# kit4b/kit4b

Measured on AMD Instinct MI355X. Metric: Mreads/sec aligned (100 bp SE vs 3 Gbp .sfx), higher is better.
Workload: dtype u64

## Files before the change

kit4b_amd/__init__.py:

```python
import ctypes as C
import os
import subprocess

import numpy as np

PKG_DIR = os.path.dirname(os.path.abspath(__file__))
LIB_PATH = os.path.join(PKG_DIR, os.environ.get("K4SFX_LIB_NAME", "libk4sfx.so"))

STRAND_BOTH, STRAND_WATSON, STRAND_CRICK = 0, 1, 2
HR_NONE, HR_HITS, HR_MMDELTA, HR_HITINSTS, HR_RMMDELTA, HR_SEQERRS = 0, 1, 2, 3, 4, 5
NAR_ACCEPTED, NAR_NS, NAR_NOHIT, NAR_MMDELTA, NAR_MULTIALIGN = 1, 2, 3, 4, 5

HIT_DTYPE = np.dtype(
    [("chrom_id", "<u4"), ("match_loci", "<u4"), ("match_len", "<u2"), ("strand", "u1"), ("mismatches", "u1"),
     ("reserved", "<u4")]
)
RESULT_DTYPE = np.dtype(
    [("hit_rslt", "<i4"), ("inst", "<i4"), ("low_mm", "<i4"), ("nxt_mm", "<i4"), ("nar", "<i4"), ("num_hits", "<i4")]
)
EXT_CHIMERIC, EXT_INDEL, EXT_INSERT, EXT_SPLICE, EXT_NONORPHAN = 1 << 24, 1 << 25, 1 << 26, 1 << 27, 1 << 28
SEG2_DTYPE = np.dtype(
    [("chrom_id", "<u4"), ("match_loci", "<u4"), ("match_len", "<u2"), ("read_ofs", "<u2"), ("mismatches", "u1"),
     ("reserved", "u1"), ("score", "<u2")]
)
# ... 231 lines not shown
                                        C.POINTER(u64), C.POINTER(SamStats), vp, vp]
    L.k4_format_bam_dev.argtypes = [vp, i32, i64, vp, vp, C.c_int32, vp, vp, vp, vp, vp, C.POINTER(SamNames), C.c_int32, C.POINTER(vp),
                                    C.POINTER(u64), C.POINTER(SamStats), vp, vp]
    L.k4_pipeline_format_bam.argtypes = [vp, C.c_int32, C.POINTER(SamStats), vp, C.POINTER(u64)]
    L.k4_pipeline_open.argtypes = [vp, C.POINTER(PipelineParams), C.POINTER(vp)]
    L.k4_pipeline_acquire.argtypes = [vp, i32, C.POINTER(vp), C.POINTER(u64)]
    L.k4_pipeline_submit.argtypes = [vp, i32, u64, i32]
    L.k4_pipeline_submit_host.argtypes = [vp, i32, vp, u64, i32]
    L.k4_pipeline_wait_aligned.argtypes = [vp, C.POINTER(PipelineView)]
    L.k4_pipeline_format.argtypes = [vp, C.POINTER(SamStats), vp, C.POINTER(u64)]
    L.k4_pipeline_next_sam.argtypes = [vp, C.POINTER(vp), C.POINTER(u64)]
    L.k4_pipeline_read_sam.argtypes = [vp, vp, u64, C.POINTER(u64)]
    L.k4_pipeline_close.argtypes = [vp]
    L.k4_pipeline_close.restype = None
    L.k4_free_device.argtypes = [vp]
    L.k4_free_device.restype = None
    L.k4_alloc_device.argtypes = [vp, u64, C.POINTER(vp)]
    L.k4_copy_to_device.argtypes = [vp, vp, vp, u64]
    L.k4_copy_to_host.argtypes = [vp, vp, vp, u64]
    L.k4_upload_pageable.argtypes = [i32, vp, vp, u64]
    L.k4_host_register.argtypes = [vp, u64]
    L.k4_host_unregister.argtypes = [vp]
    dbl, pvp, pu64 = C.c_double, C.POINTER(vp), C.POINTER(u64)
    fmt_head = [vp, i32, i64, vp, vp, C.c_int32, vp, vp, vp, vp, vp, C.POINTER(SamNames)]
    L.k4_format_sam_all_dev.argtypes = fmt_head + [pvp, pu64, C.POINTER(SamStats), vp, vp]
    L.k4_format_bam_all_dev.argtypes = fmt_head + [C.c_int32, pvp, pu64, C.POINTER(SamStats), vp, vp]
    L.k4_pipeline_format_all.argtypes = [vp, C.POINTER(SamStats), vp, pu64]
    L.k4_pipeline_format_bam_all.argtypes = [vp, C.c_int32, C.POINTER(SamStats), vp, pu64]
    L.k4_pipeline_set_trims.argtypes = [vp, C.c_int32, C.c_int32]
    L.k4_pipeline_set_sampling.argtypes = [vp, C.c_int32]
    L.k4_unaligned_fasta_dev.argtypes = [vp, i32, i64, vp, vp, vp, vp, vp, C.POINTER(SamNames), C.c_int32, pvp, pu64, pu64, vp]
    L.k4_prepare_reads_trim_dev.argtypes = [vp, i32, i64, C.c_int32, C.c_int32, C.c_int32, C.c_int32, C.c_int32, i64, vp, vp, vp, vp, u64,
                                            vp, vp, pu64, pu64, C.POINTER(u32), vp]
    snp_head = [vp, i32, i64, vp, vp, C.c_int32, vp, vp, vp, vp, C.c_int32, dbl, dbl]
    L.k4_snp_csv_dev.argtypes = snp_head + [pvp, pu64, pu64, vp]
    L.k4_snp_vcf_dev.argtypes = snp_head + [pvp, pu64, pu64, vp]
    L.k4_snp_files_dev.argtypes = [vp, i32] + snp_head[1:] + [pvp, pu64, pu64, pvp, pu64, vp]
    L.k4_snp_run_dev.argtypes = [vp, i32] + snp_head[1:] + [vp, vp]
    L.k4_snp_run2_dev.argtypes = [vp, i32] + snp_head[1:] + [C.POINTER(SnpOpts), C.POINTER(SnpFiles2), vp]
    L.k4_marker_classify_host.argtypes = [vp, u64, u32, vp, C.c_int32, dbl, vp, vp]
    L.k4_free_host.argtypes = [vp]
    L.k4_free_host.restype = None
    L.k4_pba_run_dev.argtypes = [vp, i32, i64, vp, vp, C.c_int32, vp, vp, vp, vp, C.c_char_p, C.c_char_p, C.POINTER(PbaFiles), vp]
    L.k4_pba_classify_host.argtypes = [vp, u64, u32, vp, vp, vp]
    L.k4_sfx_map.argtypes = [C.c_char_p, vp]
    L.k4_sfx_unmap.argtypes = [vp]
    L.k4_sfx_unmap.restype = None
    L.k4_set_raw_header.argtypes = [vp, vp]
    L.k4_set_description.argtypes = [vp, C.c_char_p, C.c_char_p]
    L.k4_get_sfx_header.argtypes = [vp, vp]
    L.k4_abi_version.argtypes = []
    L.k4_global_error.argtypes = []
    L.k4_get_kernel_times_split.argtypes = [vp, C.POINTER(dbl), C.POINTER(dbl), C.POINTER(C.c_int32)]
    _lib = L
    return L


def _flatten(reads):
    if isinstance(reads, tuple):
        cat, offs, lens = reads
        return (np.ascontiguousarray(cat, dtype=np.uint8), np.ascontiguousarray(offs, dtype=np.uint64),
                np.ascontiguousarray(lens, dtype=np.uint32))
    lens = np.array([len(r) for r in reads], dtype=np.uint32)
    offs = np.zeros(len(reads), dtype=np.uint64)
    if len(reads):
        offs[1:] = np.cumsum(lens[:-1], dtype=np.uint64)
        cat = np.ascontiguousarray(np.concatenate(reads).astype(np.uint8))
    else:
        cat = np.zeros(0, dtype=np.uint8)
    return cat, offs, lens


def gen_hash16(name):
    if not name:
        return 0
    h = 19937
    for ch in name.lower():
        h = ((h ^ ch) * 3119) & 0xFFFFFFFF
        if h & 0x80000000:
            h -= 1 << 32
        h ^= h >> 13
        h &= 0xFFFF
    return h or 19937


def make_entries(names, lens):
    arr = (Entry * len(names))()
    ofs = 0
    for i, (nm, ln) in enumerate(zip(names, lens)):
        arr[i].entry_id = i + 1
        arr[i].fblock_id = 1
        arr[i].name = nm.encode() if isinstance(nm, str) else nm
        arr[i].name_hash = gen_hash16(arr[i].name)
        arr[i].seq_len = int(ln)
        arr[i].start_ofs = ofs
        arr[i].end_ofs = ofs + int(ln) - 1
        ofs += int(ln) + 1
    return arr


class SfxIndex:

    def __init__(self, handle):
        self.h = C.c_void_p(handle)
        self._keep = []

# ... 40 lines not shown
    def info(self):
        o = Info()
        self._ck(lib().k4_info(self.h, C.byref(o)))
        return {f[0]: (getattr(o, f[0]).decode() if f[0] == "dataset" else getattr(o, f[0])) for f in Info._fields_}

    def entry(self, entry_id):
        e = Entry()
        self._ck(lib().k4_get_entry(self.h, entry_id, C.byref(e)))
        return dict(entry_id=e.entry_id, name=e.name.decode(), seq_len=e.seq_len, start_ofs=e.start_ofs,
                    end_ofs=e.end_ofs)

    def get_ident(self, name):
        return lib().k4_get_ident(self.h, name.encode())

    def set_max_iter(self, it):
        return lib().k4_set_max_iter(self.h, it)

    def set_fastq_quality(self, method):
        self._ck(lib().k4_set_fastq_quality(self.h, method))

    def get_seq(self, entry_id, loci, length):
        out = np.zeros(length, dtype=np.uint8)
        n = lib().k4_get_seq(self.h, entry_id, loci, out.ctypes.data, length)
        return out[:n]

    def write_sfx(self, path):
        self._ck(lib().k4_write_sfx(self.h, path.encode()))

    def min_core_len(self, pmode=0):
        s = C.c_int(0)
        m = self._ck(lib().k4_min_core_len(self.h, pmode, C.byref(s)))
        return m, s.value

    def counters(self):
        c = Counters()
        self._ck(lib().k4_get_counters(self.h, C.byref(c)))
        return {f[0]: getattr(c, f[0]) for f in Counters._fields_}

    def reset_counters(self):
        self._ck(lib().k4_reset_counters(self.h))

    def enable_kernel_timing(self, on=True):
        self._ck(lib().k4_enable_kernel_timing(self.h, 1 if on else 0))

    def kernel_times(self):
        ms, n = C.c_double(0), C.c_int32(0)
        self._ck(lib().k4_get_kernel_times(self.h, C.byref(ms), C.byref(n)))
        return ms.value, n.value

    def kernel_times_split(self):
        ms, g, n = C.c_double(0), C.c_double(0), C.c_int32(0)
        self._ck(lib().k4_get_kernel_times_split(self.h, C.byref(ms), C.byref(g), C.byref(n)))
        return ms.value, g.value, n.value

    def reserve(self, max_reads, max_read_len, max_hits):
        self._ck(lib().k4_reserve(self.h, max_reads, max_read_len, max_hits))

    def align_reads_batch(self, reads, tot_mm, core_len, core_delta, max_slides, min_core_len=0, mm_delta=1,
                          strand=STRAND_BOTH, max_hits=1):
        cat, offs, lens = _flatten(reads)
        n = len(lens)
        p = AlignParams(tot_mm, core_len, core_delta, max_slides, min_core_len, mm_delta, strand, max_hits)
        rslt = np.zeros(n, np.int32); inst = np.zeros(n, np.int32); low = np.zeros(n, np.int32)
        nxt = np.zeros(n, np.int32)
        hits = np.zeros((n, max_hits), dtype=HIT_DTYPE)
        self._ck(lib().k4_align_reads_batch(self.h, C.byref(p), n, cat.ctypes.data, offs.ctypes.data,
                                            lens.ctypes.data, rslt.ctypes.data, inst.ctypes.data, low.ctypes.data,
                                            nxt.ctypes.data, hits.ctypes.data))
        return dict(rslt=rslt, inst=inst, low=low, nxt=nxt, hits=hits)

    def align_reads_ext_batch(self, reads, tot_mm, core_len, core_delta, max_slides, min_core_len=0, mm_delta=1,
                              strand=STRAND_BOTH, max_hits=1, min_chimeric_len=0, micro_indel_len=0, max_splice_junct_len=0):
        cat, offs, lens = _flatten(reads)
        n = len(lens)
        p = AlignParams(tot_mm, core_len, core_delta, max_slides, min_core_len, mm_delta, strand, max_hits,
                        min_chimeric_len, micro_indel_len, max_splice_junct_len)
        rslt = np.zeros(n, np.int32); inst = np.zeros(n, np.int32); low = np.zeros(n, np.int32)
        nxt = np.zeros(n, np.int32)
        hits = np.zeros((n, max_hits), dtype=HIT_DTYPE)
        seg2 = np.zeros(n, dtype=SEG2_DTYPE)
        self._ck(lib().k4_align_reads_ext_batch(self.h, C.byref(p), n, cat.ctypes.data, offs.ctypes.data, lens.ctypes.data,
                                                rslt.ctypes.data, inst.ctypes.data, low.ctypes.data, nxt.ctypes.data,
                                                hits.ctypes.data, seg2.ctypes.data))
        return dict(rslt=rslt, inst=inst, low=low, nxt=nxt, hits=hits, seg2=seg2)

    def kalign_ext_batch(self, reads, max_subs=5, min_edit_dist=1, max_ns=1, pmode=0, strand=STRAND_BOTH, max_ml=1,
                         pe_mode=0, min_core_len=0, max_num_slides=0, min_chimeric_len=0, micro_indel_len=0,
                         max_splice_junct_len=0):
        cat, offs, lens = _flatten(reads)
        n = len(lens)
        p = KalignParams(max_subs, min_edit_dist, max_ns, pmode, strand, max_ml, pe_mode, min_core_len, max_num_slides,
                         min_chimeric_len, micro_indel_len, max_splice_junct_len)
        out = np.zeros(n, dtype=RESULT_DTYPE)
        hits = np.zeros((n, max(1, max_ml)), dtype=HIT_DTYPE)
        seg2 = np.zeros(n, dtype=SEG2_DTYPE)
        self._ck(lib().k4_kalign_ext_batch(self.h, C.byref(p), n, cat.ctypes.data, offs.ctypes.data, lens.ctypes.data,
                                           out.ctypes.data, hits.ctypes.data, seg2.ctypes.data))
        return dict(out=out, hits=hits, seg2=seg2)

    def best_matches_batch(self, reads, tot_mm, core_len, core_delta, max_core_slides, strand=STRAND_BOTH, max_hits=5):
        cat, offs, lens = _flatten(reads)
        n = len(lens)
        p = AlignParams(tot_mm, core_len, core_delta, max_core_slides, 0, 1, strand, max_hits)
        rslt = np.zeros(n, dtype=np.int32)
        inst = np.zeros(n, dtype=np.int32)
        hits = np.zeros((n, max_hits), dtype=HIT_DTYPE)
# ... 473 lines not shown
```

kit4b_amd/csrc/k4_align.hip:

```cpp
#include <stdlib.h>
#include <type_traits>
#include "k4_align_common.h"

#define K4_BS(nch) ((nch) >= 16 ? 128 : 256)
template <int NCH>
struct K4Lane {
  const uint64_t* rd;
  uint32_t* ded;
  const uint32_t* sup;
  const uint64_t* ent;
  uint64_t* memo;
  static constexpr int NW = NCH + 1;
  K4_DEV uint64_t word(int s, int c) const { return rd[(s * NW + c) * K4_BS(NCH)]; }
  K4_DEV uint64_t chunk_at(int s, int o) const {
    int w = o >> 5, sh = 2 * (o & 31);
    uint64_t hi = word(s, w);
    if (!sh) return hi;
    return (hi << sh) | (word(s, w + 1) >> (64 - sh));
  }
};

struct K4Probe {
  int cmp;
  int mm;
// ... 273 lines not shown
    if (32 * c < len) {
      uint32_t dq[9] = {0, 0, 0, 0, 0, 0, 0, 0, 0};
      if (c * 32 + 32 <= span) {
        uint32_t d8[8];
        k4d_load_words<8>(src32 + c * 8, d8);
#pragma unroll
        for (int q = 0; q < 8; q++) dq[q] = d8[q];
      } else {
#pragma unroll
        for (int q = 0; q < 8; q++)
          if (c * 32 + q * 4 < span) dq[q] = src32[c * 8 + q];
      }
      if (c * 32 + 32 < span) dq[8] = src32[c * 8 + 8];
#pragma unroll
      for (int q = 0; q < 8; q++) {
        const int base = c * 32 + q * 4;
        uint32_t d = __builtin_amdgcn_alignbyte(dq[q + 1], dq[q], sh);
        d &= 0x07070707u;
        if (base + 4 > len) d &= len > base ? (0xFFFFFFFFu >> (8 * (4 - (len - base)))) : 0u;
        const uint32_t hi4 = d & 0x04040404u;
        if (hi4) {
          const uint32_t inval = hi4 & ((d << 1) | (d << 2)) & 0x04040404u;
          if (inval) fl |= K4_RF_INVALID;
          n_ns += __popc(hi4 & ~inval);
          d &= ~(hi4 | (hi4 >> 1) | (hi4 >> 2));
        }
        acc = (acc << 8) | ((d & 3) << 6) | (((d >> 8) & 3) << 4) | (((d >> 16) & 3) << 2) | ((d >> 24) & 3);
      }
    }
    col[c * K4_BS(NCH)] = acc;
  }
  col[NCH * K4_BS(NCH)] = 0;
  if (n_ns) fl |= K4_RF_HAS_N;
#pragma unroll
  for (int c = 0; c < NCH; c++) {
    uint64_t r = 0;
    if (32 * c < len) {
      const int o = len - 32 * (c + 1);
      uint64_t f;
      if (o >= 0) {
        const int w = o >> 5, sh = 2 * (o & 31);
        const uint64_t hi = col[w * K4_BS(NCH)];
        f = sh ? (hi << sh) | (col[(w + 1) * K4_BS(NCH)] >> (64 - sh)) : hi;
      } else
        f = col[0] >> (2 * (-o));
      r = k4d_rev2(~f) & k4d_range_mask(0, len - 32 * c);
    }
    col[(NW + c) * K4_BS(NCH)] = r;
  }
  col[(NW + NCH) * K4_BS(NCH)] = 0;
  return fl;
}

template <int EL, int NCH, bool FIRST, typename KT, bool DEFER = false>
__global__ void __launch_bounds__(K4_BS(NCH), (NCH >= 16 ? K4_STEP_WAVES_LONG : NCH >= 8 ? K4_STEP_WAVES_MID : NCH == 5 ? K4_STEP_WAVES_5 : K4_STEP_WAVES)) k4k_align_step(K4AlignArgs a, int step, const uint32_t* __restrict__ in_ids,
                                                      const uint64_t* __restrict__ in_rows,
                                                      const uint32_t* __restrict__ in_count, uint32_t* __restrict__ out_ids,
                                                      uint64_t* __restrict__ out_rows, uint32_t* __restrict__ out_count) {
  extern __shared__ uint64_t lds[];
  constexpr int NW = NCH + 1;
  const int tid = threadIdx.x;
  const int lane = tid & 63;
  K4Lane<NCH> ln;
  ln.rd = lds + tid;
  ln.ded = reinterpret_cast<uint32_t*>(lds + 2 * NW * K4_BS(NCH)) + tid;
  ln.memo = lds + 2 * NW * K4_BS(NCH) + (K4_DEDUP_CAP * K4_BS(NCH)) / 2 + tid;
  uint64_t* ent_l = lds + 2 * NW * K4_BS(NCH) + (K4_DEDUP_CAP * K4_BS(NCH)) / 2 + 2 * K4_BS(NCH);
  uint32_t* sup_l = reinterpret_cast<uint32_t*>(ent_l + 2 * K4_LDS_ENTRIES);
  ln.ent = ent_l;
  ln.sup = sup_l;
  for (int q = tid; q < K4_SUP_WORDS; q += K4_BS(NCH)) sup_l[q] = a.ix.excsup[q];
  if (a.ix.n_entries <= K4_LDS_ENTRIES)
    for (int q = tid; q < (int)a.ix.n_entries; q += K4_BS(NCH)) {
      ent_l[q] = a.ix.ent_start[q];
      ent_l[K4_LDS_ENTRIES + q] = a.ix.ent_end[q];
    }
  __syncthreads();
  uint64_t* col = lds + tid;
  uint32_t n_lookup = 0, n_probe = 0, n_cand = 0, n_slow = 0, n_bases = 0, n_done = 0;
  const int64_t count = (FIRST && !(DEFER && in_ids != nullptr)) ? a.n_reads : (int64_t)*in_count;
  const int64_t stride = (int64_t)gridDim.x * K4_BS(NCH);
  uint32_t ch_cur = 0, ch_left = 0;
  const bool from_list = !FIRST || (DEFER && in_ids != nullptr);
  const bool may_defer = DEFER && FIRST && in_ids == nullptr && a.defer_ids != nullptr;
  uint32_t dch_cur = 0, dch_left = 0;
  for (int64_t jb = (int64_t)blockIdx.x * K4_BS(NCH) + (tid & ~63); jb < count; jb += stride) {
    const int64_t j = jb + lane;
    bool active = j < count;
    int64_t i = 0;
    if (active) {
      i = from_list ? (int64_t)in_ids[j] : j;
      if (from_list && (uint32_t)i == K4_NO_READ) active = false;
    }
    bool slow = false, survive = false, deferred = false;
    int ext_from = -1;
    if (active) {
      const int len = (int)a.lens[i];
      const K4ReadParams rp = k4d_read_params(a, len);
      bool skip = false;
      if (FIRST) {
        if (!from_list) {
          n_done++;
          n_bases += (uint32_t)len;
        }
        uint32_t fl = 0, n_ns = 0;
        if (len < 1 || len > 32 * NCH || len > K4_MAX_FAST_READ_LEN) {
          fl = K4_RF_TOOLONG;
          if (a.mode == 1) {
            const uint8_t* src = a.reads + a.offs[i];
            for (int q = 0; q < len; q++) {
              uint32_t b = src[q] & 7;
              if (b == 4) n_ns++; else if (b > 4) fl |= K4_RF_INVALID;
            }
          }
        } else
          fl = k4d_pack_read<NCH>(a.reads + a.offs[i], len, col, n_ns);
        if (a.mode == 1) {
          int max_ns = 0;
          if (a.kp.max_ns) max_ns = max((len * a.kp.max_ns) / 100, a.kp.max_ns);
          if ((fl & K4_RF_INVALID) || (int)n_ns > max_ns) {
            k4_read_result r = {K4_HR_SEQERRS, 0, 0, 0, K4_NAR_NS, 0};
            a.rr[i] = r;
            if (!a.sparse_hits)
              for (int q = 0; q < a.max_hits; q++) *reinterpret_cast<uint4*>(&a.hits[i * a.max_hits + q]) = make_uint4(0, 0, 0, 0);
            skip = true;
          }
        }
        slow = fl != 0 && !skip;
        if (((a.mode == 1 && a.kp.pe_mode == 4) || a.best) && !skip) slow = true;
      } else {
        const uint64_t* row = in_rows + (int64_t)j * K4_ROW_WORDS(NCH);
        {
          const k4_u64x2_a8 mv = *reinterpret_cast<const k4_u64x2_a8*>(row + 2 * NCH);
          ln.memo[0] = mv.x; ln.memo[K4_BS(NCH)] = mv.y;
        }
        uint64_t rw[2 * NCH];
#pragma unroll
        for (int c = 0; c < NCH; c++) {
          const k4_u64x2_a8 v = *reinterpret_cast<const k4_u64x2_a8*>(row + 2 * c);
          rw[2 * c] = v.x; rw[2 * c + 1] = v.y;
        }
#pragma unroll
        for (int c = 0; c < NCH; c++) {
          col[c * K4_BS(NCH)] = rw[c];
          col[(NW + c) * K4_BS(NCH)] = rw[NCH + c];
        }
        col[NCH * K4_BS(NCH)] = 0;
        col[(NW + NCH) * K4_BS(NCH)] = 0;
      }
      if (!skip && (rp.core_len < 1 || rp.max_hits < 1 || rp.max_hits > a.max_hits)) slow = true;
      if (!skip && !slow) {
        int n_esc = 0;
        if (rp.tot_mm > 0)
          for (; n_esc <= rp.tot_mm; n_esc++)
            if (len / (n_esc + rp.mm_delta) <= rp.core_len) break;
        const bool has_final = rp.tot_mm > 0 ? n_esc <= rp.tot_mm : true;
        const int n_phases = n_esc + (has_final ? 1 : 0);
        int allow, cl, delta;
        if (step < n_esc) { allow = step; cl = len / (step + rp.mm_delta); delta = cl; }
        else { allow = rp.tot_mm; cl = rp.core_len; delta = rp.core_delta; }
        k4_hit* hits = a.hits + i * a.max_hits;
        int inst = 0, low = 0, nxt = 0;
        const uint32_t c0 = n_lookup, c1 = n_probe, c2 = n_cand;
        if (FIRST) { ln.memo[0] = K4_MEMO_NONE; ln.memo[K4_BS(NCH)] = K4_MEMO_NONE; }
        int rslt = k4d_lcm_fast<EL, NCH, KT, FIRST>(a, ln, len, allow, cl, delta, rp, &inst, &low, &nxt, hits, n_lookup, n_probe, n_cand, DEFER && may_defer);
        if (rslt == K4_NEED_SLOW) {
          slow = true;
          n_lookup = c0; n_probe = c1; n_cand = c2;
        }
        else if (DEFER && rslt == K4_DEFER) {
          deferred = true;
          n_lookup = c0; n_probe = c1; n_cand = c2;
        }
        else if (rslt == 0 && step + 1 >= n_phases && a.ext_on) { slow = true; ext_from = n_phases; }
        else if (rslt != 0 || step + 1 >= n_phases) k4d_finalize(a, i, len, rp, rslt, inst, low, nxt);
        else survive = true;
      }
      if (slow) {
        k4d_push_slow(a, i, ext_from >= 0 ? ext_from : step);
        n_slow++;
      }
    }
    if (FIRST && DEFER) {
      const unsigned long long dm = __ballot(deferred);
      const uint32_t dcnt = (uint32_t)__popcll(dm);
      if (dcnt) {
        if (dcnt > dch_left) {
          for (uint32_t q = lane; q < dch_left; q += 64) a.defer_ids[dch_cur + q] = K4_NO_READ;
          uint32_t base = 0;
          if (lane == 0) base = atomicAdd(&a.ctl[K4_CTL_DEFER], (uint32_t)K4_CHUNK);
          dch_cur = __shfl(base, 0, 64);
          dch_left = K4_CHUNK;
        }
        if (deferred) a.defer_ids[dch_cur + (uint32_t)__popcll(dm & ((1ull << lane) - 1ull))] = (uint32_t)i;
        dch_cur += dcnt;
        dch_left -= dcnt;
      }
    }
    const unsigned long long m = __ballot(survive);
    const uint32_t cnt = (uint32_t)__popcll(m);
    if (cnt) {
      if (cnt > ch_left) {
        for (uint32_t q = lane; q < ch_left; q += 64) out_ids[ch_cur + q] = K4_NO_READ;
        uint32_t base = 0;
        if (lane == 0) base = atomicAdd(out_count, (uint32_t)K4_CHUNK);
        ch_cur = __shfl(base, 0, 64);
        ch_left = K4_CHUNK;
      }
      if (survive) {
        const uint32_t slot = ch_cur + (uint32_t)__popcll(m & ((1ull << lane) - 1ull));
        out_ids[slot] = (uint32_t)i;
        uint64_t* row = out_rows + (int64_t)slot * K4_ROW_WORDS(NCH);
#pragma unroll
// ... 56 lines not shown
  int fast_len = std::min<int>(max_read_len, K4_MAX_FAST_READ_LEN);
  if (max_reads > w.cap_reads || fast_len > w.cap_len) {
    int64_t cap = std::max<int64_t>(max_reads, w.cap_reads);
    cap = (cap + 255) / 256 * 256;
    int len = std::max(fast_len, w.cap_len);
    int nch = nch_for(len);
    touched = true;
    w.cap_reads = 0;
    w.cap_len = 0;
    const size_t slots = k4_survivor_slots((size_t)cap);
    for (int b = 0; b < 2; b++) {
      K4_HIP(ix, w.ids[b].reserve(slots * 4));
      K4_HIP(ix, w.rows[b].reserve(slots * K4_ROW_WORDS(nch) * 8));
    }
    K4_HIP(ix, w.slow_list.reserve((size_t)cap * 4));
    K4_HIP(ix, w.slow_step.reserve((size_t)cap));
    K4_HIP(ix, w.huge_list.reserve((size_t)cap * 4));
    K4_HIP(ix, w.huge_step.reserve((size_t)cap));
    w.cap_reads = cap;
    w.cap_len = len;
  }
  if (!w.ctl.p) {
    touched = true;
    K4_HIP(ix, w.ctl.reserve(K4_CTL_WORDS * 4));
    K4_HIP(ix, hipMemset(w.ctl.p, 0, K4_CTL_WORDS * 4));
  }
  uint64_t nodes = ix->d.max_iter ? std::min<uint64_t>((uint64_t)ix->d.max_iter * 48, K4_MAX_IDENT_NODES) : K4_MAX_IDENT_NODES;
  uint32_t hcap = next_pow2(std::max<uint64_t>(2 * nodes + 2, 1024));
  if (!w.slow_hash.p || hcap > w.slow_hash_cap) {
    touched = true;
    const size_t words = (size_t)K4_SLOW_WAVES * K4_SMALL_HASH + (size_t)K4_HUGE_WAVES * hcap;
    const size_t bytes = words * 8 + (size_t)(K4_SLOW_WAVES + K4_HUGE_WAVES) * 4;
    K4_HIP(ix, w.slow_hash.reserve(bytes));
    K4_HIP(ix, hipMemset(w.slow_hash.p, 0, bytes));
    w.slow_hash_cap = hcap;
  }
  w.cap_hits = std::max(w.cap_hits, max_hits);
  if (touched) K4_HIP(ix, hipDeviceSynchronize());
  return K4_OK;
}

template <int EL, int NCH, typename KT>
static int launch_steps(k4_index* ix, K4AlignArgs& a, int n_steps, hipStream_t st) {
  K4Workspace& w = ix->ws;
  uint32_t* const ids[2] = {w.ids[0].as<uint32_t>(), w.ids[1].as<uint32_t>()};
  uint64_t* const rows[2] = {w.rows[0].as<uint64_t>(), w.rows[1].as<uint64_t>()};
  uint32_t* const ctl = w.ctl.as<uint32_t>();
  const size_t lds = (size_t)2 * (NCH + 1) * K4_BS(NCH) * 8 + (size_t)K4_DEDUP_CAP * K4_BS(NCH) * 4 + (size_t)2 * K4_BS(NCH) * 8 + (size_t)2 * K4_LDS_ENTRIES * 8 +
                     (size_t)K4_SUP_WORDS * 4 + 16;
  if (lds > 48 * 1024) {
    K4_HIP(ix, hipFuncSetAttribute((const void*)k4k_align_step<EL, NCH, true, KT, false>, hipFuncAttributeMaxDynamicSharedMemorySize, (int)lds));
    K4_HIP(ix, hipFuncSetAttribute((const void*)k4k_align_step<EL, NCH, true, KT, true>, hipFuncAttributeMaxDynamicSharedMemorySize, (int)lds));
    K4_HIP(ix, hipFuncSetAttribute((const void*)k4k_align_step<EL, NCH, false, KT>, hipFuncAttributeMaxDynamicSharedMemorySize, (int)lds));
  }
  const unsigned full = 256 * 8 * (256 / K4_BS(NCH));
  const bool timed = ix->timing && ix->ev_used < 4096;
  if (timed) {
    if (ix->ev_used == ix->ev0.size()) {
      hipEvent_t e0, e1, e2;
      K4_HIP(ix, hipEventCreate(&e0));
      K4_HIP(ix, hipEventCreate(&e1));
      K4_HIP(ix, hipEventCreate(&e2));
      ix->ev0.push_back(e0);
      ix->ev1.push_back(e1);
      ix->ev2.push_back(e2);
    }
    K4_HIP(ix, hipEventRecord(ix->ev0[ix->ev_used], st));
  }
  unsigned grid0 = (unsigned)std::min<int64_t>((a.n_reads + K4_BS(NCH) - 1) / K4_BS(NCH), full);
  static const int deep_mode = getenv("K4_DEEP_TO_GENERAL") ? atoi(getenv("K4_DEEP_TO_GENERAL")) : 0;
  a.deep_general = (deep_mode && ix->deep_bucket_frac >= K4_DEFER_MIN_FRAC) ? deep_mode : 0;
  if (ix->deep_bucket_frac >= K4_DEFER_MIN_FRAC && a.deep_general != 1) {
    a.defer_ids = ids[1];
    hipLaunchKernelGGL((k4k_align_step<EL, NCH, true, KT, true>), dim3(grid0), dim3(K4_BS(NCH)), lds, st, a, 0, (const uint32_t*)nullptr,
                       (const uint64_t*)nullptr, (const uint32_t*)nullptr, ids[0], rows[0], ctl + 2);
    hipLaunchKernelGGL((k4k_align_step<EL, NCH, true, KT, true>), dim3(grid0), dim3(K4_BS(NCH)), lds, st, a, 0, (const uint32_t*)ids[1],
                       (const uint64_t*)nullptr, (const uint32_t*)(ctl + K4_CTL_DEFER), ids[0], rows[0], ctl + 2);
  } else {
    a.defer_ids = nullptr;
    hipLaunchKernelGGL((k4k_align_step<EL, NCH, true, KT, false>), dim3(grid0), dim3(K4_BS(NCH)), lds, st, a, 0, (const uint32_t*)nullptr,
                       (const uint64_t*)nullptr, (const uint32_t*)nullptr, ids[0], rows[0], ctl + 2);
  }
  for (int t = 1; t < n_steps; t++) {
    const int in = (t - 1) & 1, out = t & 1;
    hipLaunchKernelGGL((k4k_align_step<EL, NCH, false, KT>), dim3(grid0), dim3(K4_BS(NCH)), lds, st, a, t, ids[in], rows[in],
                       ctl + 2 + (t - 1), ids[out], rows[out], ctl + 2 + t);
  }
  if (timed) K4_HIP(ix, hipEventRecord(ix->ev1[ix->ev_used], st));
  return K4_OK;
}

template <int EL, typename KT>
static int launch_all(k4_index* ix, K4AlignArgs& a, int max_len, int n_steps, hipStream_t st) {
  K4Workspace& w = ix->ws;
  const int nch = nch_for(std::min(max_len, K4_MAX_FAST_READ_LEN));
  if (nch > nch_for(w.cap_len)) return k4_fail(ix, K4_ERR_INTERNAL, "workspace not reserved for read length %d", max_len);
  if (n_steps < 1 || n_steps > K4_CTL_WORDS - 4) return k4_fail(ix, K4_ERR_INTERNAL, "bad phase count %d", n_steps);
  a.slow_list = w.slow_list.as<uint32_t>();
  a.slow_step = w.slow_step.as<uint8_t>();
  a.ctl = w.ctl.as<uint32_t>();
  a.counters = ix->counters.as<unsigned long long>();
  a.huge_list = w.huge_list.as<uint32_t>();
  a.huge_step = w.huge_step.as<uint8_t>();
  a.slow_hash = w.slow_hash.as<uint64_t>();
  a.slow_hash_cap = w.slow_hash_cap;
  a.slow_gen = reinterpret_cast<uint32_t*>(a.slow_hash + (size_t)K4_SLOW_WAVES * K4_SMALL_HASH + (size_t)K4_HUGE_WAVES * w.slow_hash_cap);
  a.nw = nch + 1;
  if (a.n_reads == 0) return K4_OK;
  K4_HIP(ix, hipMemsetAsync(w.ctl.p, 0, K4_CTL_WORDS * 4, st));
  int rc;
  switch (nch) {
    case 4: rc = launch_steps<EL, 4, KT>(ix, a, n_steps, st); break;
    case 5: rc = launch_steps<EL, 5, KT>(ix, a, n_steps, st); break;
    case 8: rc = launch_steps<EL, 8, KT>(ix, a, n_steps, st); break;
    default: rc = launch_steps<EL, 16, KT>(ix, a, n_steps, st); break;
  }
  if (rc != K4_OK) return rc;
  rc = k4i_launch_general(ix, a, max_len, st);
  if (rc != K4_OK) return rc;
  if (ix->timing && ix->ev_used < ix->ev0.size() && ix->ev_used < 4096) {
    K4_HIP(ix, hipEventRecord(ix->ev2[ix->ev_used], st));
    ix->ev_used++;
  }
  K4_HIP(ix, hipGetLastError());
  return K4_OK;
}

static int run_dev(k4_index* ix, K4AlignArgs& a, int max_len, void* stream) {
  K4Workspace& w = ix->ws;
  if (a.n_reads > w.cap_reads || std::min(max_len, K4_MAX_FAST_READ_LEN) > w.cap_len || a.max_hits > w.cap_hits ||
      !w.slow_hash.p || !w.ids[0].p || !w.ids[1].p || !w.rows[0].p || !w.rows[1].p || !w.slow_list.p || !w.huge_list.p || !w.ctl.p)
    return k4_fail(ix, K4_ERR_PARAMS, "k4_reserve(%lld, %d, %d) must precede the *_dev call", (long long)a.n_reads,
                   max_len, a.max_hits);
  a.ix = ix->d;
  hipStream_t st = (hipStream_t)stream;
  {
    const int mc = a.mode == 0 ? a.ap.min_chimeric_len : a.kp.min_chimeric_len;
    const int mi = a.mode == 0 ? a.ap.micro_indel_len : a.kp.micro_indel_len;
    const int ms = a.mode == 0 ? a.ap.max_splice_junct_len : a.kp.max_splice_junct_len;
    if (mc < 0 || mi < 0 || mi > 20 || ms < 0 || (ms != 0 && (ms < 25 || ms > 100000)))
      return k4_fail(ix, K4_ERR_PARAMS, "MinChimericLen / microInDelLen (0..20) / MaxSpliceJunctLen (0, 25..100000) out of range");
    a.ext_on = (mc > 0 || mi > 0 || ms > 0) ? 1 : 0;
    if ((mi > 0 || ms > 0) && !a.seg2)
      return k4_fail(ix, K4_ERR_PARAMS, "microInDel / splice phases report two segments: use the *_ext entry points (k4_seg2 output)");
    if (a.ext_on && (a.best || (a.mode == 1 && a.kp.pe_mode == 4)))
      return k4_fail(ix, K4_ERR_PARAMS, "the optional AlignReads phases cannot be combined with LocateBestMatches (-N)");
    if (a.seg2 && a.n_reads > 0) K4_HIP(ix, hipMemsetAsync(a.seg2, 0, (size_t)a.n_reads * sizeof(k4_seg2), st));
  }
  int tot_mm = a.ap.tot_mm;
  if (a.mode == 1) {
    tot_mm = a.kp.max_subs == 0 ? 0 : std::max(1, (int)(0.5 + (max_len * a.kp.max_subs) / 100.0));
    tot_mm = std::min(tot_mm, 63);
  }
  const int n_steps = tot_mm + 1;
  if (ix->d.el == 4) return ix->d.ktab64 ? launch_all<4, uint64_t>(ix, a, max_len, n_steps, st) : launch_all<4, uint32_t>(ix, a, max_len, n_steps, st);
  return ix->d.ktab64 ? launch_all<5, uint64_t>(ix, a, max_len, n_steps, st) : launch_all<5, uint32_t>(ix, a, max_len, n_steps, st);
}

static int check_align_params(k4_index* ix, const k4_align_params* p) {
  if (!p) return K4_ERR_PARAMS;
  if (p->tot_mm < 0 || p->tot_mm > 63 || p->core_len < 1 || p->core_delta < 0 || p->max_core_slides < 1 ||
      p->mm_delta < 1 || p->strand < 0 || p->strand > 2 || p->max_hits < 1 || p->max_hits > 4096)
// ... 236 lines not shown
  if (seg2) K4_HIP(ix, s2.alloc((size_t)n * sizeof(k4_seg2)));
  rc = k4_kalign_ext_batch_dev(ix, p, n, max_len, w.c_reads, w.c_offs, w.c_lens, w.c_out, w.c_hits, s2.p, ix->stream);
  if (rc != K4_OK) return rc;
  if (seg2 && (rc = seg2_fetch(ix, seg2, s2, n)) != K4_OK) return rc;
  return stage_out(ix, n, p->max_ml, {out}, sizeof(k4_read_result), hits);
}

extern "C" int k4_enable_kernel_timing(k4_index* ix, int on) {
  if (!ix) return K4_ERR_PARAMS;
  ix->timing = on != 0;
  return K4_OK;
}

extern "C" int k4_get_kernel_times_split(k4_index* ix, double* step_ms, double* general_ms, int32_t* launches) {
  if (!ix || !step_ms || !general_ms || !launches) return K4_ERR_PARAMS;
  K4_HIP(ix, hipSetDevice(ix->device));
  K4_HIP(ix, hipDeviceSynchronize());
  double tot = 0, tot_g = 0;
  for (size_t j = 0; j < ix->ev_used; j++) {
    float ms = 0;
    K4_HIP(ix, hipEventElapsedTime(&ms, ix->ev0[j], ix->ev1[j]));
    tot += ms;
    K4_HIP(ix, hipEventElapsedTime(&ms, ix->ev1[j], ix->ev2[j]));
    tot_g += ms;
  }
  *step_ms = tot;
  *general_ms = tot_g;
  *launches = (int32_t)ix->ev_used;
  ix->ev_used = 0;
  return K4_OK;
}
extern "C" int k4_get_kernel_times(k4_index* ix, double* fast_ms, int32_t* launches) {
  double g = 0;
  return k4_get_kernel_times_split(ix, fast_ms, &g, launches);
}

extern "C" int k4_get_counters(k4_index* ix, k4_counters* out) {
  if (!ix || !out) return K4_ERR_PARAMS;
  K4_HIP(ix, hipSetDevice(ix->device));
  K4_HIP(ix, hipDeviceSynchronize());
  K4_HIP(ix, hipMemcpy(out, ix->counters.p, sizeof(k4_counters), hipMemcpyDeviceToHost));
  return K4_OK;
}

extern "C" int k4i_debug_prof(k4_index* ix, uint64_t* out) {
  if (!ix || !out) return K4_ERR_PARAMS;
  K4_HIP(ix, hipSetDevice(ix->device));
  K4_HIP(ix, hipDeviceSynchronize());
  K4_HIP(ix, hipMemcpy(out, ix->counters.as<char>() + sizeof(k4_counters), K4_PROF_SLOTS * 8, hipMemcpyDeviceToHost));
  K4_HIP(ix, hipMemset(ix->counters.as<char>() + sizeof(k4_counters), 0, K4_PROF_SLOTS * 8));
  return K4_OK;
}

extern "C" int k4_reset_counters(k4_index* ix) {
  if (!ix) return K4_ERR_PARAMS;
  K4_HIP(ix, hipSetDevice(ix->device));
  K4_HIP(ix, hipDeviceSynchronize());
  K4_HIP(ix, hipMemset(ix->counters.p, 0, sizeof(k4_counters)));
  return K4_OK;
}
```

kit4b_amd/csrc/k4_align_common.h:

```cpp
#pragma once
#include <stdio.h>
#include <string.h>
#include <algorithm>
#include "k4_device.h"

#define K4_NEED_SLOW (-100)
#define K4_DEFER (-101)
#define K4_RF_HAS_N 1u
#define K4_RF_INVALID 2u
#define K4_RF_TOOLONG 4u
#ifndef K4_STEP_WAVES
#define K4_STEP_WAVES 4
#endif
#ifndef K4_STEP_WAVES_LONG
#define K4_STEP_WAVES_LONG 2
#endif
#ifndef K4_STEP_WAVES_5
#define K4_STEP_WAVES_5 4
#endif
#ifndef K4_STEP_WAVES_MID
#define K4_STEP_WAVES_MID 3
#endif
#define K4_CHUNK 512
#define K4_NO_READ 0xFFFFFFFFu
#define K4_ROW_WORDS(nch) (2 * (nch) + 2)
#ifndef K4_PF
#define K4_PF 4
#endif
#ifndef K4_PF5
#define K4_PF5 4
#endif
#ifndef K4_SLOW_WAVES_PER_EU
#define K4_SLOW_WAVES_PER_EU 4
#endif
#ifndef K4_SLOW_WAVES_PER_EU_EXT
#define K4_SLOW_WAVES_PER_EU_EXT 3
#endif
#ifndef K4_DEFER_BUCKET
#define K4_DEFER_BUCKET K4_DEEP_BUCKET
#endif
#define K4_DEFER_MIN_FRAC 0.002
#ifndef K4_SLOW_KB
#define K4_SLOW_KB 1
#endif
#ifndef K4_SLOW_WAVES
#define K4_SLOW_WAVES 8192
#endif
#define K4_SMALL_HASH 4096
#define K4_HUGE_WAVES 256
#define K4_CTL_HUGE 68
#define K4_CTL_DEFER 70
#define K4_CTL_WORDS 72

struct K4AlignArgs {
  K4DevIndex ix;
  const uint8_t* reads;
  const uint64_t* offs;
  const uint32_t* lens;
  int64_t n_reads;
  int32_t mode;
  int32_t sparse_hits;
  int32_t best;
  int32_t deep_general;
  k4_align_params ap;
  k4_kalign_params kp;
  int32_t* rslt;
  int32_t* inst;
  int32_t* low;
  int32_t* nxt;
  k4_read_result* rr;
  k4_hit* hits;
  k4_seg2* seg2;
  int32_t ext_on;
  int32_t max_hits;
  uint32_t* slow_list;
  uint8_t* slow_step;
  uint32_t* huge_list;
  uint8_t* huge_step;
  uint32_t* defer_ids;
  uint32_t* ctl;
  unsigned long long* counters;
  uint64_t* slow_hash;
  uint32_t* slow_gen;
  uint32_t slow_hash_cap;
  int32_t nw;
};

struct K4ReadParams {
  int tot_mm, core_len, core_delta, max_slides, mm_delta, strand, max_hits;
  int min_core_len, min_chimeric_len, micro_indel_len, max_splice_junct_len;
};

struct K4State {
  int inst, low, nxt, cur_hit;
};

K4_DEV K4ReadParams k4d_read_params(const K4AlignArgs& a, int len) {
  K4ReadParams p;
  if (a.mode == 0) {
    p.tot_mm = a.ap.tot_mm; p.core_len = a.ap.core_len; p.core_delta = a.ap.core_delta;
    p.max_slides = a.ap.max_core_slides; p.mm_delta = a.ap.mm_delta; p.strand = a.ap.strand;
    p.max_hits = a.ap.max_hits;
    p.min_core_len = a.ap.min_core_len; p.min_chimeric_len = a.ap.min_chimeric_len;
    p.micro_indel_len = a.ap.micro_indel_len; p.max_splice_junct_len = a.ap.max_splice_junct_len;
    return p;
  }
  int mm = a.kp.max_subs == 0 ? 0 : (int)(0.5 + (len * a.kp.max_subs) / 100.0);
  if (a.kp.max_subs != 0 && mm < 1) mm = 1;
  if (mm > 63) mm = 63;
  int cl = len / (a.kp.min_edit_dist == 1 ? mm + 1 : mm + 2);
  if (cl < a.kp.min_core_len) cl = a.kp.min_core_len;
  int sl = (a.kp.max_num_slides * len + 99) / 100;
  if (sl < 1) sl = 1;
  int cd = len / sl - 1;
  if (cd < cl) cd = cl;
// ... 89 lines not shown
```

kit4b_amd/csrc/k4_internal.h:

```cpp
#pragma once
#include <hip/hip_runtime.h>
#include <stdint.h>
#include <string>
#include <thread>
#include <vector>
#include "../../include/k4sfx.h"
#include "k4_pool.h"

#define K4_EXC_SHIFT 8
#define K4_EXC_BLOCK (1 << K4_EXC_SHIFT)
#define K4_SUP_WORDS 512
#define K4_LDS_ENTRIES 128
#define K4_PAD_BASES 2048
#define K4_PAD_WORDS (K4_PAD_BASES / 16)
#define K4_MAX_FAST_READ_LEN 512
#define K4_MAX_READ_LEN 4096
#define K4_PROF_SLOTS 32
#ifndef K4_DEEP_BUCKET
#define K4_DEEP_BUCKET 24
#endif
#define K4_DEDUP_CAP 6
#define K4_MAX_IDENT_NODES 1024000

struct K4DevIndex {
  const uint32_t* ref2;
  const uint32_t* excbm;
  const uint32_t* excsup;
  const uint32_t* excblk;
  const uint32_t* excnib;
  const uint8_t* sa;
  const void* ktab;
  const uint64_t* ent_start;
  const uint64_t* ent_end;
  const uint32_t* ent_id;
  uint64_t n;
  uint32_t n_exc;
  uint32_t n_entries;
  uint32_t el;
  uint32_t k;
  uint32_t ktab64;
  uint32_t sup_shift;
  int32_t max_iter;
};

struct K4Workspace {
  int64_t cap_reads = 0;
  int32_t cap_len = 0;
  int32_t cap_hits = 0;
  K4DevBuf ids[2];
  K4DevBuf rows[2];
  K4DevBuf slow_list;
  K4DevBuf slow_step;
  K4DevBuf huge_list;
  K4DevBuf huge_step;
  K4DevBuf ctl;
  K4DevBuf slow_hash;
  uint32_t slow_hash_cap = 0;
  K4DevBuf d_reads, d_offs, d_lens;
  K4DevBuf d_out4;
  K4DevBuf d_hits;
  int64_t stage_reads = 0; int32_t stage_hits = 0;
  uint8_t* h_small = nullptr;
  K4DevBuf d_small;
  const uint8_t* c_reads = nullptr; const uint64_t* c_offs = nullptr; const uint32_t* c_lens = nullptr;
  int32_t* c_out = nullptr; k4_hit* c_hits = nullptr; bool c_small = false;
};

struct k4_index {
  int device = 0;
  K4DevIndex d{};
  K4DevBuf ref2, excbm, excsup, excblk, excnib, sa, ktab, ent_start, ent_end, ent_id;
  K4DevBuf counters;
  int q_method = 3;
  K4DevBuf d_qlut;
  K4DevBuf d_run_stats;
  uint64_t filter_prior[20] = {0};
  double deep_bucket_frac = 0;
  std::vector<k4_entry> entries;
  std::string dataset;
  std::string description, title;
  std::vector<uint8_t> raw_header;
  uint64_t tot_seqs_len = 0;
  uint64_t device_bytes = 0;
  std::string err;
  K4Workspace ws;
  K4DevBuf pe_rr, pe_hits, pe_list, pe_ctl;
  int64_t pe_cap_pairs = 0;
  int32_t pe_cap_hits = 0;
  K4DevBuf rs_tasks, rs_reads, rs_res, rs_hits;
  std::thread loader;
  int load_rc = 0;
  double load_seconds = 0;
  hipStream_t stream = nullptr;
  bool timing = false;
  std::vector<hipEvent_t> ev0, ev1, ev2;
  size_t ev_used = 0;
};

void k4_set_global_error(const char* fmt, ...);
int k4_fail(k4_index* ix, int code, const char* fmt, ...);
int k4_check_hip(k4_index* ix, hipError_t e, const char* what);

int k4i_build_device_structures(k4_index* ix, const void* d_seq_bytes, int kmer_k);
#define K4_SMALL_STAGE (4u << 20)
#define K4_SMALL_READS 4096
int k4i_kalign_batch_dev(k4_index* ix, const k4_kalign_params* p, int64_t n, int32_t max_len, const void* d_reads,
                         const void* d_offs, const void* d_lens, void* d_out, void* d_hits, void* stream, int sparse_hits);
int k4i_stats_tally_multi(k4_index* ix, const void* d_rr, int64_t n, void* stream);
unsigned long long* k4i_stats_pe_len_dist(k4_index* ix);
int k4i_build_sa(uint64_t n, uint32_t el, const uint8_t* d_seq, uint8_t* d_sa, int device, std::string* err);

#define K4_HIP(ix, call)                                   \
  do {                                                     \
    int _rc = k4_check_hip((ix), (call), #call);           \
    if (_rc != K4_OK) return _rc;                          \
  } while (0)
```

Before: 3093.

## Add uniform-read-length kernel variant selected on device by length span

Adds a small kernel that computes the min and max read length on the device and writes them into the control block, replacing the memset. Each align step is launched twice, once as a uniform-length specialization and once as the general version. Each launch exits early unless the span matches its variant. The uniform variant hoists the per-read length load, parameter derivation and phase planning out of the per-lane loop. The cost is double kernel launches with early-exit blocks and an extra reduction kernel per batch.

```diff
diff --git a/kit4b_amd/__init__.py b/kit4b_amd/__init__.py
--- a/kit4b_amd/__init__.py
+++ b/kit4b_amd/__init__.py
@@ -307,6 +307,8 @@
     L.k4_abi_version.argtypes = []
     L.k4_global_error.argtypes = []
     L.k4_get_kernel_times_split.argtypes = [vp, C.POINTER(dbl), C.POINTER(dbl), C.POINTER(C.c_int32)]
+    if hasattr(L, "k4i_set_uniform_len_mode"):
+        L.k4i_set_uniform_len_mode.argtypes = [vp, i32]
     _lib = L
     return L
 
@@ -453,6 +455,9 @@
         ms, g, n = C.c_double(0), C.c_double(0), C.c_int32(0)
         self._ck(lib().k4_get_kernel_times_split(self.h, C.byref(ms), C.byref(g), C.byref(n)))
         return ms.value, g.value, n.value
+
+    def set_uniform_len_mode(self, mode=-1):
+        return self._ck(lib().k4i_set_uniform_len_mode(self.h, mode))
 
     def reserve(self, max_reads, max_read_len, max_hits):
         self._ck(lib().k4_reserve(self.h, max_reads, max_read_len, max_hits))
diff --git a/kit4b_amd/csrc/k4_align.hip b/kit4b_amd/csrc/k4_align.hip
--- a/kit4b_amd/csrc/k4_align.hip
+++ b/kit4b_amd/csrc/k4_align.hip
@@ -349,7 +349,56 @@
   return fl;
 }
 
-template <int EL, int NCH, bool FIRST, typename KT, bool DEFER = false>
+struct K4Plan {
+  int n_phases, allow, cl, delta;
+};
+K4_DEV K4Plan k4d_phase_plan(const K4ReadParams& rp, int len, int step) {
+  K4Plan pl;
+  int n_esc = 0;
+  if (rp.tot_mm > 0)
+    for (; n_esc <= rp.tot_mm; n_esc++)
+      if (len / (n_esc + rp.mm_delta) <= rp.core_len) break;
+  const bool has_final = rp.tot_mm > 0 ? n_esc <= rp.tot_mm : true;
+  pl.n_phases = n_esc + (has_final ? 1 : 0);
+  if (step < n_esc) { pl.allow = step; pl.cl = len / (step + rp.mm_delta); pl.delta = pl.cl; }
+  else { pl.allow = rp.tot_mm; pl.cl = rp.core_len; pl.delta = rp.core_delta; }
+  return pl;
+}
+
+#define K4_SPAN_BS 256
+__global__ void __launch_bounds__(K4_SPAN_BS) k4k_ctl_span(const uint32_t* __restrict__ lens, int64_t n, uint32_t* __restrict__ ctl) {
+  if (blockIdx.x == 0)
+    for (int q = threadIdx.x; q < K4_CTL_WORDS; q += K4_SPAN_BS)
+      if (q < K4_CTL_LEN_MIN || q == K4_CTL_PATH) ctl[q] = 0;
+  uint32_t nlo = 0, hi = 0;
+  const int64_t stride = (int64_t)gridDim.x * K4_SPAN_BS;
+  for (int64_t j = (int64_t)blockIdx.x * K4_SPAN_BS + threadIdx.x; j < n; j += stride) {
+    const uint32_t v = lens[j];
+    nlo = max(nlo, ~v);
+    hi = max(hi, v);
+  }
+  for (int d = 32; d > 0; d >>= 1) {
+    nlo = max(nlo, (uint32_t)__shfl_down(nlo, d, 64));
+    hi = max(hi, (uint32_t)__shfl_down(hi, d, 64));
+  }
+  __shared__ uint32_t part[2][K4_SPAN_BS / 64];
+  if ((threadIdx.x & 63) == 0) { part[0][threadIdx.x >> 6] = nlo; part[1][threadIdx.x >> 6] = hi; }
+  __syncthreads();
+  if (threadIdx.x == 0) {
+    for (int q = 1; q < K4_SPAN_BS / 64; q++) { nlo = max(nlo, part[0][q]); hi = max(hi, part[1][q]); }
+    atomicMax(&ctl[K4_CTL_SPAN_ACC], nlo);
+    atomicMax(&ctl[K4_CTL_SPAN_ACC + 1], hi);
+    __threadfence();
+    if (atomicAdd(&ctl[K4_CTL_SPAN_ACC + 2], 1u) == gridDim.x - 1) {
+      __threadfence();
+      ctl[K4_CTL_LEN_MIN] = ~atomicExch(&ctl[K4_CTL_SPAN_ACC], 0u);
+      ctl[K4_CTL_LEN_MAX] = atomicExch(&ctl[K4_CTL_SPAN_ACC + 1], 0u);
+      ctl[K4_CTL_SPAN_ACC + 2] = 0;
+    }
+  }
+}
+
+template <int EL, int NCH, bool FIRST, typename KT, bool DEFER = false, bool UNI = false>
 __global__ void __launch_bounds__(K4_BS(NCH), (NCH >= 16 ? K4_STEP_WAVES_LONG : NCH >= 8 ? K4_STEP_WAVES_MID : NCH == 5 ? K4_STEP_WAVES_5 : K4_STEP_WAVES)) k4k_align_step(K4AlignArgs a, int step, const uint32_t* __restrict__ in_ids,
                                                       const uint64_t* __restrict__ in_rows,
                                                       const uint32_t* __restrict__ in_count, uint32_t* __restrict__ out_ids,
@@ -357,6 +406,11 @@
   extern __shared__ uint64_t lds[];
   constexpr int NW = NCH + 1;
   const int tid = threadIdx.x;
+  if (a.uni_select) {
+    const uint32_t lo = __builtin_amdgcn_readfirstlane(a.ctl[K4_CTL_LEN_MIN]), hi = __builtin_amdgcn_readfirstlane(a.ctl[K4_CTL_LEN_MAX]);
+    if ((lo == hi) != UNI) return;
+  }
+  if (blockIdx.x == 0 && tid == 0) atomicOr(&a.ctl[K4_CTL_PATH], UNI ? 1u : 2u);
   const int lane = tid & 63;
   K4Lane<NCH> ln;
   ln.rd = lds + tid;
@@ -381,6 +435,14 @@
   const bool from_list = !FIRST || (DEFER && in_ids != nullptr);
   const bool may_defer = DEFER && FIRST && in_ids == nullptr && a.defer_ids != nullptr;
   uint32_t dch_cur = 0, dch_left = 0;
+  int u_len = 0;
+  K4ReadParams u_rp = {};
+  K4Plan u_pl = {};
+  if (UNI) {
+    u_len = __builtin_amdgcn_readfirstlane((int)a.ctl[K4_CTL_LEN_MAX]);
+    u_rp = k4d_read_params(a, u_len);
+    u_pl = k4d_phase_plan(u_rp, u_len, step);
+  }
   for (int64_t jb = (int64_t)blockIdx.x * K4_BS(NCH) + (tid & ~63); jb < count; jb += stride) {
     const int64_t j = jb + lane;
     bool active = j < count;
@@ -392,8 +454,8 @@
     bool slow = false, survive = false, deferred = false;
     int ext_from = -1;
     if (active) {
-      const int len = (int)a.lens[i];
-      const K4ReadParams rp = k4d_read_params(a, len);
+      const int len = UNI ? u_len : (int)a.lens[i];
+      const K4ReadParams rp = UNI ? u_rp : k4d_read_params(a, len);
       bool skip = false;
       if (FIRST) {
         if (!from_list) {
@@ -447,15 +509,8 @@
       }
       if (!skip && (rp.core_len < 1 || rp.max_hits < 1 || rp.max_hits > a.max_hits)) slow = true;
       if (!skip && !slow) {
-        int n_esc = 0;
-        if (rp.tot_mm > 0)
-          for (; n_esc <= rp.tot_mm; n_esc++)
-            if (len / (n_esc + rp.mm_delta) <= rp.core_len) break;
-        const bool has_final = rp.tot_mm > 0 ? n_esc <= rp.tot_mm : true;
-        const int n_phases = n_esc + (has_final ? 1 : 0);
-        int allow, cl, delta;
-        if (step < n_esc) { allow = step; cl = len / (step + rp.mm_delta); delta = cl; }
-        else { allow = rp.tot_mm; cl = rp.core_len; delta = rp.core_delta; }
+        const K4Plan pl = UNI ? u_pl : k4d_phase_plan(rp, len, step);
+        const int n_phases = pl.n_phases, allow = pl.allow, cl = pl.cl, delta = pl.delta;
         k4_hit* hits = a.hits + i * a.max_hits;
         int inst = 0, low = 0, nxt = 0;
         const uint32_t c0 = n_lookup, c1 = n_probe, c2 = n_cand;
@@ -618,6 +673,9 @@
     K4_HIP(ix, hipFuncSetAttribute((const void*)k4k_align_step<EL, NCH, true, KT, false>, hipFuncAttributeMaxDynamicSharedMemorySize, (int)lds));
     K4_HIP(ix, hipFuncSetAttribute((const void*)k4k_align_step<EL, NCH, true, KT, true>, hipFuncAttributeMaxDynamicSharedMemorySize, (int)lds));
     K4_HIP(ix, hipFuncSetAttribute((const void*)k4k_align_step<EL, NCH, false, KT>, hipFuncAttributeMaxDynamicSharedMemorySize, (int)lds));
+    K4_HIP(ix, hipFuncSetAttribute((const void*)k4k_align_step<EL, NCH, true, KT, false, true>, hipFuncAttributeMaxDynamicSharedMemorySize, (int)lds));
+    K4_HIP(ix, hipFuncSetAttribute((const void*)k4k_align_step<EL, NCH, true, KT, true, true>, hipFuncAttributeMaxDynamicSharedMemorySize, (int)lds));
+    K4_HIP(ix, hipFuncSetAttribute((const void*)k4k_align_step<EL, NCH, false, KT, false, true>, hipFuncAttributeMaxDynamicSharedMemorySize, (int)lds));
   }
   const unsigned full = 256 * 8 * (256 / K4_BS(NCH));
   const bool timed = ix->timing && ix->ev_used < 4096;
@@ -636,19 +694,32 @@
   unsigned grid0 = (unsigned)std::min<int64_t>((a.n_reads + K4_BS(NCH) - 1) / K4_BS(NCH), full);
   static const int deep_mode = getenv("K4_DEEP_TO_GENERAL") ? atoi(getenv("K4_DEEP_TO_GENERAL")) : 0;
   a.deep_general = (deep_mode && ix->deep_bucket_frac >= K4_DEFER_MIN_FRAC) ? deep_mode : 0;
+  const bool uni = a.uni_select != 0;
   if (ix->deep_bucket_frac >= K4_DEFER_MIN_FRAC && a.deep_general != 1) {
     a.defer_ids = ids[1];
+    if (uni)
+      hipLaunchKernelGGL((k4k_align_step<EL, NCH, true, KT, true, true>), dim3(grid0), dim3(K4_BS(NCH)), lds, st, a, 0, (const uint32_t*)nullptr,
+                         (const uint64_t*)nullptr, (const uint32_t*)nullptr, ids[0], rows[0], ctl + 2);
     hipLaunchKernelGGL((k4k_align_step<EL, NCH, true, KT, true>), dim3(grid0), dim3(K4_BS(NCH)), lds, st, a, 0, (const uint32_t*)nullptr,
                        (const uint64_t*)nullptr, (const uint32_t*)nullptr, ids[0], rows[0], ctl + 2);
+    if (uni)
+      hipLaunchKernelGGL((k4k_align_step<EL, NCH, true, KT, true, true>), dim3(grid0), dim3(K4_BS(NCH)), lds, st, a, 0, (const uint32_t*)ids[1],
+                         (const uint64_t*)nullptr, (const uint32_t*)(ctl + K4_CTL_DEFER), ids[0], rows[0], ctl + 2);
     hipLaunchKernelGGL((k4k_align_step<EL, NCH, true, KT, true>), dim3(grid0), dim3(K4_BS(NCH)), lds, st, a, 0, (const uint32_t*)ids[1],
                        (const uint64_t*)nullptr, (const uint32_t*)(ctl + K4_CTL_DEFER), ids[0], rows[0], ctl + 2);
   } else {
     a.defer_ids = nullptr;
+    if (uni)
+      hipLaunchKernelGGL((k4k_align_step<EL, NCH, true, KT, false, true>), dim3(grid0), dim3(K4_BS(NCH)), lds, st, a, 0, (const uint32_t*)nullptr,
+                         (const uint64_t*)nullptr, (const uint32_t*)nullptr, ids[0], rows[0], ctl + 2);
     hipLaunchKernelGGL((k4k_align_step<EL, NCH, true, KT, false>), dim3(grid0), dim3(K4_BS(NCH)), lds, st, a, 0, (const uint32_t*)nullptr,
                        (const uint64_t*)nullptr, (const uint32_t*)nullptr, ids[0], rows[0], ctl + 2);
   }
   for (int t = 1; t < n_steps; t++) {
     const int in = (t - 1) & 1, out = t & 1;
+    if (uni)
+      hipLaunchKernelGGL((k4k_align_step<EL, NCH, false, KT, false, true>), dim3(grid0), dim3(K4_BS(NCH)), lds, st, a, t, ids[in], rows[in],
+                         ctl + 2 + (t - 1), ids[out], rows[out], ctl + 2 + t);
     hipLaunchKernelGGL((k4k_align_step<EL, NCH, false, KT>), dim3(grid0), dim3(K4_BS(NCH)), lds, st, a, t, ids[in], rows[in],
                        ctl + 2 + (t - 1), ids[out], rows[out], ctl + 2 + t);
   }
@@ -661,7 +732,8 @@
   K4Workspace& w = ix->ws;
   const int nch = nch_for(std::min(max_len, K4_MAX_FAST_READ_LEN));
   if (nch > nch_for(w.cap_len)) return k4_fail(ix, K4_ERR_INTERNAL, "workspace not reserved for read length %d", max_len);
-  if (n_steps < 1 || n_steps > K4_CTL_WORDS - 4) return k4_fail(ix, K4_ERR_INTERNAL, "bad phase count %d", n_steps);
+  static_assert(K4_CTL_MAX_STEPS >= 64 && 2 + K4_CTL_MAX_STEPS <= K4_CTL_HUGE, "ctl[2 + t] holds the survivors of up to 64 phases");
+  if (n_steps < 1 || n_steps > K4_CTL_MAX_STEPS) return k4_fail(ix, K4_ERR_INTERNAL, "bad phase count %d", n_steps);
   a.slow_list = w.slow_list.as<uint32_t>();
   a.slow_step = w.slow_step.as<uint8_t>();
   a.ctl = w.ctl.as<uint32_t>();
@@ -673,7 +745,11 @@
   a.slow_gen = reinterpret_cast<uint32_t*>(a.slow_hash + (size_t)K4_SLOW_WAVES * K4_SMALL_HASH + (size_t)K4_HUGE_WAVES * w.slow_hash_cap);
   a.nw = nch + 1;
   if (a.n_reads == 0) return K4_OK;
-  K4_HIP(ix, hipMemsetAsync(w.ctl.p, 0, K4_CTL_WORDS * 4, st));
+  a.uni_select = ix->uniform_len_mode != 0;
+  {
+    const unsigned blocks = (unsigned)std::min<int64_t>((a.n_reads + 4 * K4_SPAN_BS - 1) / (4 * K4_SPAN_BS), 2048);
+    hipLaunchKernelGGL(k4k_ctl_span, dim3(blocks), dim3(K4_SPAN_BS), 0, st, a.lens, a.n_reads, a.ctl);
+  }
   int rc;
   switch (nch) {
     case 4: rc = launch_steps<EL, 4, KT>(ix, a, n_steps, st); break;
@@ -1016,6 +1092,17 @@
   return K4_OK;
 }
 
+extern "C" int k4i_set_uniform_len_mode(k4_index* ix, int mode) {
+  if (!ix || mode > 1) return K4_ERR_PARAMS;
+  if (mode >= 0) ix->uniform_len_mode = mode;
+  if (!ix->ws.ctl.p) return 0;
+  K4_HIP(ix, hipSetDevice(ix->device));
+  K4_HIP(ix, hipDeviceSynchronize());
+  uint32_t path = 0;
+  K4_HIP(ix, hipMemcpy(&path, ix->ws.ctl.as<uint32_t>() + K4_CTL_PATH, 4, hipMemcpyDeviceToHost));
+  return (int)path;
+}
+
 extern "C" int k4_reset_counters(k4_index* ix) {
   if (!ix) return K4_ERR_PARAMS;
   K4_HIP(ix, hipSetDevice(ix->device));
diff --git a/kit4b_amd/csrc/k4_align_common.h b/kit4b_amd/csrc/k4_align_common.h
--- a/kit4b_amd/csrc/k4_align_common.h
+++ b/kit4b_amd/csrc/k4_align_common.h
@@ -50,7 +50,12 @@
 #define K4_HUGE_WAVES 256
 #define K4_CTL_HUGE 68
 #define K4_CTL_DEFER 70
-#define K4_CTL_WORDS 72
+#define K4_CTL_LEN_MIN 72
+#define K4_CTL_LEN_MAX 73
+#define K4_CTL_SPAN_ACC 74
+#define K4_CTL_PATH 77
+#define K4_CTL_WORDS 80
+#define K4_CTL_MAX_STEPS (K4_CTL_HUGE - 2)
 
 struct K4AlignArgs {
   K4DevIndex ix;
@@ -61,6 +66,7 @@
   int32_t mode;
   int32_t sparse_hits;
   int32_t best;
+  int32_t uni_select;
   int32_t deep_general;
   k4_align_params ap;
   k4_kalign_params kp;
diff --git a/kit4b_amd/csrc/k4_internal.h b/kit4b_amd/csrc/k4_internal.h
--- a/kit4b_amd/csrc/k4_internal.h
+++ b/kit4b_amd/csrc/k4_internal.h
@@ -1,6 +1,7 @@
 #pragma once
 #include <hip/hip_runtime.h>
 #include <stdint.h>
+#include <stdlib.h>
 #include <string>
 #include <thread>
 #include <vector>
@@ -66,8 +67,14 @@
   int32_t* c_out = nullptr; k4_hit* c_hits = nullptr; bool c_small = false;
 };
 
+inline int k4i_env_uniform_len() {
+  const char* e = getenv("K4_UNIFORM_LEN");
+  return (e && *e) ? (atoi(e) != 0 ? 1 : 0) : 1;
+}
+
 struct k4_index {
   int device = 0;
+  int uniform_len_mode = k4i_env_uniform_len();
   K4DevIndex d{};
   K4DevBuf ref2, excbm, excsup, excblk, excnib, sa, ktab, ent_start, ent_end, ent_id;
   K4DevBuf counters;
```

New measurement: 3145 (median of 6 runs). +1.7%, better.
